# bridgedp/hunter_bipedal_control

Hardware: AMD Instinct MI355X
Metric: MPC+WBC updates/sec (batch=4096, N=100, 12-DoF) (higher is better)
Workload: dtype f64; 1 GPU; 4096 distinct hunter instances (4096/GPU, state seed 1234 + id), trot gait from t = 0.1, cmd_vel (0.3, 0, 0, 0), N=100 shooting intervals (dt 0.015 s), node tables generated on the device (hb_refgen_update, per-knot IK joint references), 1 SQP iteration + WeightedWbc per update, x0 of every call perturbed by measurement noise (sigma 0.01) so that no call re-solves a converged problem: every line s; batch_per_gpu=4096, total_instances=4096, horizon_nodes=100

## Files before the change

### hunter_bipedal_control_amd/abi.py

```python
from __future__ import annotations

import ctypes as C
from types import SimpleNamespace

import numpy as np

NX, NU, NV, NJ, NC, NBODY, NWBC, NRBD, SWING_REF = 22, 22, 16, 10, 4, 11, 38, 32, 6
FLY, MODE_R, MODE_L, STANCE = 0, 1, 2, 3
HB_PAYLOAD_SIZE = 10
HB_PROFILE_MAX_KNOTS = 16
HB_PROFILE_RECORD = 10


class HbModel(C.Structure):
    _fields_ = [
        ("parent", C.c_int32 * NJ),
        ("joint_origin", (C.c_double * 3) * NJ),
        ("joint_axis", (C.c_double * 3) * NJ),
        ("q_lower", C.c_double * NJ), ("q_upper", C.c_double * NJ),
        ("qd_limit", C.c_double * NJ), ("effort", C.c_double * NJ),
        ("mass", C.c_double * NBODY),
        ("com", (C.c_double * 3) * NBODY),
        ("inertia", (C.c_double * 6) * NBODY),
        ("contact_body", C.c_int32 * NC),
        ("contact_offset", (C.c_double * 3) * NC),
        ("gravity", C.c_double),
    ]


class HbConfig(C.Structure):
    _fields_ = [
        ("dt", C.c_double),
        ("sqp_iterations", C.c_int32), ("wbc_type", C.c_int32),
        ("g_max", C.c_double), ("g_min", C.c_double),
        ("alpha_decay", C.c_double), ("alpha_min", C.c_double), ("gamma_c", C.c_double), ("armijo_factor", C.c_double),
        ("Q_diag", C.c_double * NX),
        ("R_task_diag", C.c_double * 24),
        ("initial_state", C.c_double * NX),
        ("friction_mu", C.c_double), ("friction_reg", C.c_double), ("friction_gripper", C.c_double),
        ("friction_hess_shift", C.c_double),
        ("friction_barrier_mu", C.c_double), ("friction_barrier_delta", C.c_double),
        ("soft_swing_weight", C.c_double),
        ("pos_limit_barrier", C.c_double * 2), ("vel_limit_barrier", C.c_double * 2),
        ("force_limit_barrier", C.c_double * 2), ("force_limit", C.c_double * 2),
        ("position_error_gain", C.c_double),
        ("zero_vel_z_gain", C.c_double), ("zero_vel_z_offset", C.c_double),
        ("xy_ref_gain", C.c_double),
        ("torque_limits", C.c_double * 5),
        ("wbc_friction_mu", C.c_double),
        ("swing_kp", C.c_double), ("swing_kd", C.c_double),
        ("base_height_kp", C.c_double), ("base_height_kd", C.c_double),
        ("base_angular_kp", C.c_double), ("base_angular_kd", C.c_double),
        ("weight_swing_leg", C.c_double), ("weight_base_accel", C.c_double), ("weight_contact_force", C.c_double),
        ("wbc_eps_reg", C.c_double),
        ("wbc_max_iter", C.c_int32), ("reserved", C.c_int32),
        ("default_joint_state", C.c_double * NJ),
        ("delta_tol", C.c_double),
        ("wbc_reg_steps", C.c_int32), ("wbc_eps_mode", C.c_int32),
    ]


_LQ = dict(LQ_LOADS=10, LQ_LEG_VALUES=6, LQ_VALUE_PREPASS=7, LQ_DIRECTIONS=9, LQ_COMPOSE=1, LQ_FACTOR=2, LQ_SOLVES=3, LQ_DEFECT=30,
           LQ_B_COLUMNS=31, LQ_COST=4, LQ_SOFT_ROWS=5, LQ_Q=32, LQ_P=33, LQ_R=34)
_WBC = dict(WBC_A_BASE=13, WBC_A_LEGS=14, WBC_A_FINISH=15, WBC_A=11, WBC_B=12)
_RIC1 = dict(RIC1_STAGING=20, RIC1_GEMM1=21, RIC1_GEMM2=22, RIC1_FACTOR=23)
_RIC4 = dict(RIC4_STAGING=24, RIC4_GEMM1=25, RIC4_GEMM2=26, RIC4_FACTOR=27)
_HWBC = dict(HWBC_LEVEL0=41, HWBC_KERNEL0=43, HWBC_QP1=44, HWBC_LEVEL1=42)
FORMS = dict(NONE=0, **_LQ, **_WBC, **_RIC1, **_RIC4, **_HWBC, RIC_BWD_ONE=101, RIC_BWD_FOUR=104, RIC_FWD_ROW=111, RIC_FWD_WAVE=114,
             LQT_ONE_RECORD=117, LQT_TRACE=118, LQT_PARK_NOTHING=119, LQT_VALUES_ONCE=125, LQT_VALUES=126, LQT_VALUES_FWD=127,
             LQT_VALUES_LEGS=128, LQ_ONE_NODE=129, LS_EVAL_NODE=151, RIC1_TRACE=197, WBC_TRACE=198, RIC4_TRACE=199)
FORM_RANGES = dict(LQ_TRIP_POW2=(120, 124), LQ_TRIP_LEN=(131, 146))
FORM = SimpleNamespace(**FORMS)
LQ_STOPS, WBC_STOPS, RIC1_STOPS, RIC4_STOPS, HWBC_STOPS = (tuple(d.values()) for d in (_LQ, _WBC, _RIC1, _RIC4, _HWBC))


class HbStats(C.Structure):
    _fields_ = [
        ("ms_lq", C.c_double), ("ms_riccati_bwd", C.c_double), ("ms_riccati_fwd", C.c_double),
        ("ms_linesearch", C.c_double), ("ms_mpc_total", C.c_double), ("ms_wbc", C.c_double),
        ("n_mpc_solves", C.c_int64), ("n_wbc_solves", C.c_int64),
        ("n_status", C.c_int32 * 4),
    ]


def _fill(arr, values):
    a = np.asarray(values)
    if a.ndim == 1:
        for i, v in enumerate(a):
            arr[i] = v.item()
    else:
        for i in range(a.shape[0]):
            for j in range(a.shape[1]):
                arr[i][j] = a[i, j].item()


def make_model(params: dict) -> HbModel:
    m = params["model"]
    out = HbModel()
    for name in ("parent", "joint_origin", "joint_axis", "q_lower", "q_upper", "qd_limit", "effort", "mass", "com",
                 "inertia", "contact_body", "contact_offset"):
        _fill(getattr(out, name), m[name])
    out.gravity = m["gravity"]
    return out


def make_config(params: dict, **overrides) -> HbConfig:
    c = params["config"]
    out = HbConfig()
    out.dt = c["dt"]
    out.sqp_iterations = c["sqp_iterations"]
    out.wbc_type = 0
    out.g_max, out.g_min = c["g_max"], c["g_min"]
    out.alpha_decay, out.alpha_min, out.gamma_c, out.armijo_factor = 0.5, 1e-4, 1e-6, 1e-4
    _fill(out.Q_diag, c["Q_diag"])
    _fill(out.R_task_diag, c["R_task_diag"])
    _fill(out.initial_state, c["initial_state"])
    out.friction_mu = c["friction_mu"]
    out.friction_reg, out.friction_gripper, out.friction_hess_shift = 25.0, 0.0, 1e-6
    out.friction_barrier_mu, out.friction_barrier_delta = c["friction_barrier_mu"], c["friction_barrier_delta"]
    out.soft_swing_weight = c["soft_swing_weight"]
    _fill(out.pos_limit_barrier, [1.0, 0.1])
    _fill(out.vel_limit_barrier, [1.0, 0.1])
    _fill(out.force_limit_barrier, [0.1, 1.0])
    _fill(out.force_limit, [0.0, 350.0])
    out.position_error_gain = c["position_error_gain"]
    out.zero_vel_z_gain, out.zero_vel_z_offset = 3.0, -0.06
    out.xy_ref_gain = 3.0
    _fill(out.torque_limits, c["torque_limits"])
    out.wbc_friction_mu = c["wbc_friction_mu"]
    out.swing_kp, out.swing_kd = c["swing_kp"], c["swing_kd"]
    out.base_height_kp, out.base_height_kd = c["base_height_kp"], c["base_height_kd"]
    out.base_angular_kp, out.base_angular_kd = c["base_angular_kp"], c["base_angular_kd"]
    out.weight_swing_leg, out.weight_base_accel = c["weight_swing_leg"], c["weight_base_accel"]
    out.weight_contact_force = c["weight_contact_force"]
    out.wbc_eps_reg = 1e-8
    out.wbc_max_iter = 120
    _fill(out.default_joint_state, c["default_joint_state"])
    out.delta_tol = c["delta_tol"]
    out.wbc_reg_steps = 1
    for k, v in overrides.items():
        if isinstance(v, (list, tuple)):
            _fill(getattr(out, k), v)
        else:
            setattr(out, k, v)
    return out


class HbEstimatorConfig(C.Structure):
    _fields_ = [(k, C.c_double) for k in (
        "foot_radius", "imu_process_noise_position", "imu_process_noise_velocity", "foot_process_noise_position",
        "foot_sensor_noise_position", "foot_sensor_noise_velocity", "foot_height_sensor_noise",
        "contact_force_cutoff_frequency", "contact_threshold")]


def make_estimator_config(params: dict, **overrides) -> HbEstimatorConfig:
    out = HbEstimatorConfig()
    for k, _ in HbEstimatorConfig._fields_:
        setattr(out, k, overrides.get(k, params["config"]["kalman"][k]))
    return out


class HbSensorConfig(C.Structure):
    _fields_ = [(k, C.c_double) for k in ("orientation_noise", "gyro_noise", "accel_noise", "joint_pos_noise", "joint_vel_noise",
                                          "joint_torque_noise")] + [("seed", C.c_uint64), ("instance_offset", C.c_uint32),
                                                                    ("reserved", C.c_int32)]


def make_sensor_config(seed: int = 0, instance_offset: int = 0, **sigmas) -> HbSensorConfig:
    out = HbSensorConfig()
    names = [k for k, _ in HbSensorConfig._fields_[:6]]
    for k, v in sigmas.items():
        if k not in names:
            raise TypeError(f"make_sensor_config: unknown channel {k!r} (one of {names})")
        setattr(out, k, float(v))
    out.seed, out.instance_offset, out.reserved = int(seed) & 0xFFFFFFFFFFFFFFFF, int(instance_offset), 0
    return out


class HbContactConfig(C.Structure):
    _fields_ = [("mode", C.c_int32), ("sweeps", C.c_int32), ("mu", C.c_double), ("ground_z", C.c_double), ("erp", C.c_double),
                ("tol", C.c_double), ("fall_height", C.c_double), ("reserved", C.c_int32 * 2)]


HB_CONTACT_NONFINITE, HB_CONTACT_FALLEN, HB_CONTACT_UNCONVERGED = 1, 2, 4
CONTACT_DEFAULT_SWEEPS = 30


def make_contact_config(params: dict, **overrides) -> HbContactConfig:
    d = dict(mode=1, sweeps=CONTACT_DEFAULT_SWEEPS, mu=params["config"]["friction_mu"], ground_z=0.0, erp=0.2, tol=1e-3, fall_height=0.0)
    for k in overrides:
        if k not in d:
            raise TypeError(f"make_contact_config: unknown field {k!r} (one of {sorted(d)})")
    d.update(overrides)
    out = HbContactConfig()
    out.mode, out.sweeps = int(d["mode"]), int(d["sweeps"])
    for k in ("mu", "ground_z", "erp", "tol", "fall_height"):
        setattr(out, k, float(d[k]))
    return out


class HbJointModel(C.Structure):
    _fields_ = [(k, C.c_double * NJ) for k in ("armature", "damping", "frictionloss", "lower", "upper", "torque_limit")] + [
        ("limit_erp", C.c_double), ("tol", C.c_double), ("limits", C.c_int32), ("reserved", C.c_int32)]


HB_JOINT_UNCONVERGED = 1 << 30


def make_joint_model(params: dict, **overrides) -> HbJointModel:
    m = params["model"]
    d = dict(armature=0.1, damping=1.0, frictionloss=0.2, lower=m["q_lower"], upper=m["q_upper"], torque_limit=100.0, limit_erp=0.2,
             tol=1e-3, limits=1)
    for k in overrides:
        if k not in d:
            raise TypeError(f"make_joint_model: unknown field {k!r} (one of {sorted(d)})")
    d.update(overrides)
    out = HbJointModel()
    for k in ("armature", "damping", "frictionloss", "lower", "upper", "torque_limit"):
        _fill(getattr(out, k), np.broadcast_to(np.asarray(d[k], dtype=float), (NJ,)))
    out.limit_erp, out.tol, out.limits, out.reserved = float(d["limit_erp"]), float(d["tol"]), int(d["limits"]), 0
    return out


# ... 254 lines not shown
```

### hunter_bipedal_control_amd/csrc/hb_forms.hpp

```cpp
#pragma once

namespace hb {
namespace form {

#define HB_FORM_CODES(X) \
  X(NONE,             0, "decode_forms",                  "the product: every form picked by the number of instances in flight") \
   \
  X(LQ_LOADS,        10, "lq_node",                       "stop: loads") \
  X(LQ_LEG_VALUES,    6, "lq_node",                       "stop: + leg value pass") \
  X(LQ_VALUE_PREPASS, 7, "lq_node",                       "stop: + value pre-pass") \
  X(LQ_DIRECTIONS,    9, "lq_node_dense",                 "stop: + direction pass (k_lq_trip: read-back of the parked image + direction pass)") \
  X(LQ_COMPOSE,       1, "lq_tail",                       "stop: + compose") \
  X(LQ_FACTOR,        2, "lq_tail",                       "stop: + Gram matrix, pivoted Cholesky") \
  X(LQ_SOLVES,        3, "lq_tail",                       "stop: + solves") \
  X(LQ_DEFECT,       30, "lq_tail",                       "stop: + defect, A~ B~ tiles") \
  X(LQ_B_COLUMNS,    31, "lq_tail",                       "stop: + B~ columns, b~") \
  X(LQ_COST,          4, "lq_tail",                       "stop: + cost") \
  X(LQ_SOFT_ROWS,     5, "lq_tail",                       "stop: + soft rows, Pj, M") \
  X(LQ_Q,            32, "lq_tail",                       "stop: + Q~ q~") \
  X(LQ_P,            33, "lq_tail",                       "stop: + P~ r~") \
  X(LQ_R,            34, "lq_tail",                       "stop: + R~ (what is left: recovery data)") \
   \
  X(WBC_A_BASE,      13, "wbc_phase_a, wbc_solve",        "stop: phase A, base pass") \
  X(WBC_A_LEGS,      14, "wbc_phase_a, wbc_solve",        "stop: + leg passes") \
  X(WBC_A_FINISH,    15, "wbc_phase_a, wbc_solve",        "stop: + composition, desired base acceleration") \
  X(WBC_A,           11, "wbc_solve",                     "stop: phase A (rigid-body quantities and fills)") \
  X(WBC_B,           12, "wbc_solve",                     "stop: + phase B (cost factor, unconstrained minimiser)") \
   \
  X(RIC1_STAGING,    20, "k_ric_bwd",                     "stop: staging of the record only") \
  X(RIC1_GEMM1,      21, "ric_phase12, k_ric_bwd",        "stop: + GEMM 1") \
  X(RIC1_GEMM2,      22, "ric_phase12, k_ric_bwd",        "stop: + GEMM 2") \
  X(RIC1_FACTOR,     23, "riccati_bwd_node, k_ric_bwd",   "stop: + factor, solves (what is left: GEMM 3)") \
   \
  X(RIC4_STAGING,    24, "k_ric_bwd4, decode_forms",      "stop: staging only") \
  X(RIC4_GEMM1,      25, "k_ric_bwd4, decode_forms",      "stop: + GEMM 1") \
  X(RIC4_GEMM2,      26, "k_ric_bwd4, decode_forms",      "stop: + GEMM 2") \
  X(RIC4_FACTOR,     27, "k_ric_bwd4, decode_forms",      "stop: + factor, solves | first part of GEMM 3") \
   \
  X(HWBC_LEVEL0,     41, "k_hwbc",                        "stop: level 0") \
  X(HWBC_KERNEL0,    43, "hwbc_solve",                    "stop: + kernel basis of level 0") \
  X(HWBC_QP1,        44, "hwbc_solve",                    "stop: + level-1 QP") \
  X(HWBC_LEVEL1,     42, "k_hwbc",                        "stop: + kernel basis of level 1 (what is left: level 2)") \
   \
  X(RIC_BWD_ONE,    101, "decode_forms",                  "selector: one-wavefront backward sweep (k_ric_bwd)") \
  X(RIC_BWD_FOUR,   104, "decode_forms",                  "selector: four-wavefront backward sweep (k_ric_bwd4)") \
  X(RIC_FWD_ROW,    111, "decode_forms",                  "selector: row form of the forward sweep (k_ric_fwd)") \
  X(RIC_FWD_WAVE,   114, "decode_forms",                  "selector: wave form of the forward sweep (k_ric_fwd_w)") \
   \
  X(LQT_ONE_RECORD, 117, "k_lq_trip",                     "stop: every node of a workgroup writes one record slot (stores issued, lines stay in the L2)") \
  X(LQT_TRACE,      118, "k_lq_trip, lq_trip_values",     "trace (-DHB_LQV_TRACE): cycle counts of workgroup 1000's value phase; the kernel returns behind it") \
  X(LQT_PARK_NOTHING, 119, "lq_park_out",                 "stop: the value phase computes but parks nothing (stale data is read back)") \
  X(LQT_VALUES_ONCE, 125, "k_lq_trip",                    "stop: the value phase runs once per trip, later launches reuse what it parked") \
  X(LQT_VALUES,     126, "k_lq_trip",                     "stop: the value phase alone (first of LQT_VALUES .. LQT_VALUES_LEGS)") \
  X(LQT_VALUES_FWD, 127, "k_lq_trip, lq_trip_values",     "stop: the value phase up to its forward sweep") \
  X(LQT_VALUES_LEGS, 128, "k_lq_trip, lq_trip_values",    "stop: the value phase up to its leg pass (last of LQT_VALUES ..)") \
  X(LQ_ONE_NODE,    129, "decode_forms",                  "selector: the one-node-per-wavefront kernel k_lq (differs from the trips by rounding)") \
   \
  X(LS_EVAL_NODE,   151, "decode_forms",                  "selector: thread-per-node line-search evaluation (k_ls_eval_node, k_ls_tail_eval_node; differs from the two-lane form by rounding)") \
   \
  X(RIC1_TRACE,     197, "k_ric_bwd",                     "trace: cycle counts of stage 50 of instance 9") \
  X(WBC_TRACE,      198, "wbc_solve, decode_forms",       "trace: cycle counts of the WeightedWbc solve of instance 5 (leaves the sweep's choice alone)") \
  X(RIC4_TRACE,     199, "k_ric_bwd4, decode_forms",      "trace: cycle counts of stage 50 of instance 7")

#define HB_FORM_RANGES(X) \
  X(LQ_TRIP_POW2,   120, 124, "decode_forms",             "selector: LQ trips of 2^(value - first) nodes") \
  X(LQ_TRIP_LEN,    131, 146, "decode_forms",             "selector: LQ trips of value - first + 1 nodes (1 .. 16)")

enum Code : int {
#define HB_FORM_ENUM(id, value, reader, meaning) id = value,
#define HB_FORM_RANGE_ENUM(id, first, last, reader, meaning) id##_FIRST = first, id##_LAST = last,
  HB_FORM_CODES(HB_FORM_ENUM) HB_FORM_RANGES(HB_FORM_RANGE_ENUM)
#undef HB_FORM_ENUM
#undef HB_FORM_RANGE_ENUM
};

struct Entry { const char* name; int first, last; const char* reader; const char* meaning; };
constexpr Entry kTable[] = {
#define HB_FORM_ROW(id, value, reader, meaning) {#id, value, value, reader, meaning},
#define HB_FORM_RANGE_ROW(id, first, last, reader, meaning) {#id, first, last, reader, meaning},
  HB_FORM_CODES(HB_FORM_ROW) HB_FORM_RANGES(HB_FORM_RANGE_ROW)
#undef HB_FORM_ROW
#undef HB_FORM_RANGE_ROW
};

}

struct KernelForms {
  enum class Bwd { Auto, One, Four } bwd = Bwd::Auto;
  enum class Fwd { Auto, Row, Wave } fwd = Fwd::Auto;
  enum class Lq { Trips, OneNode } lq = Lq::Trips;
  enum class Ls { Pair, Node } ls = Ls::Pair;
  int trip_len = 0;
};

inline KernelForms decode_forms(int reserved, bool ablate) {
  using namespace form;
  KernelForms f;
  if (reserved == RIC_BWD_FOUR) f.bwd = KernelForms::Bwd::Four;
  else if (ablate && ((reserved >= RIC4_STAGING && reserved <= RIC4_FACTOR) || reserved == RIC4_TRACE)) f.bwd = KernelForms::Bwd::Four;
  else if (reserved == RIC_BWD_ONE) f.bwd = KernelForms::Bwd::One;
  else if (ablate && reserved != NONE && reserved != WBC_TRACE) f.bwd = KernelForms::Bwd::One;
  if (reserved == RIC_FWD_WAVE) f.fwd = KernelForms::Fwd::Wave;
  else if (reserved == RIC_FWD_ROW) f.fwd = KernelForms::Fwd::Row;
  if (reserved == LQ_ONE_NODE) f.lq = KernelForms::Lq::OneNode;
  if (reserved == LS_EVAL_NODE) f.ls = KernelForms::Ls::Node;
  if (reserved >= LQ_TRIP_POW2_FIRST && reserved <= LQ_TRIP_POW2_LAST) f.trip_len = 1 << (reserved - LQ_TRIP_POW2_FIRST);
  if (reserved >= LQ_TRIP_LEN_FIRST && reserved <= LQ_TRIP_LEN_LAST) f.trip_len = reserved - LQ_TRIP_LEN_FIRST + 1;
  return f;
}

constexpr int kRicBwd4MaxBatch = 512;
inline bool use_ric_bwd4(const KernelForms& f, int concurrent) {
  return f.bwd == KernelForms::Bwd::Four || (f.bwd == KernelForms::Bwd::Auto && concurrent <= kRicBwd4MaxBatch);
}

constexpr int kRicFwdWaveMaxBatch = 512;
inline bool use_ric_fwd_wave(const KernelForms& f, int concurrent) {
  return f.fwd == KernelForms::Fwd::Wave || (f.fwd == KernelForms::Fwd::Auto && concurrent <= kRicFwdWaveMaxBatch);
}

inline bool use_ground_forms(bool map_in_force) { return map_in_force; }

struct PlantForm {
  enum class Ground { Pinned, Level, Terrain, Varied, Profile } ground;
  bool joints, hybrid;
};
inline PlantForm plant_form(int contact_mode, bool joints_on, bool terrain_on, bool modelvar_on, bool profile_on, bool hybrid) {
  using G = PlantForm::Ground;
  if (contact_mode != 1) return {G::Pinned, false, hybrid};
  return {profile_on ? G::Profile : modelvar_on ? G::Varied : terrain_on ? G::Terrain : G::Level, joints_on, hybrid};
}

constexpr int kLqTripsPerSlot = 4;
inline int lq_trip_len(const KernelForms& f, int concurrent, int Nmax, int n_cu) {
  if (f.trip_len) return f.trip_len;
  const long slots = 12L * n_cu;
  for (int sh = 4; sh > 0; --sh)
    if (long(concurrent) * ((Nmax + (1 << sh) - 1) >> sh) >= kLqTripsPerSlot * slots) return 1 << sh;
  return 1;
}

}
```

### hunter_bipedal_control_amd/csrc/hb_qpfactor.hpp

```cpp
#pragma once
#include "hb_math.hpp"

namespace hb {

template <int N>
HB_HD double dot4(const double* a, int sa, const double* b, int sb) {
  double s[4] = {0.0, 0.0, 0.0, 0.0};
#pragma unroll
  for (int i = 0; i < N; ++i) s[i & 3] += a[i * sa] * b[i * sb];
  return (s[0] + s[1]) + (s[2] + s[3]);
}

template <class Ctx>
HB_HD void givens_insert_row(const Ctx& cx, double* R, int ld, int n, double* np) {
  for (int k = 0; k < n; ++k) {
    const double a = R[k * ld + k], b = np[k];
    cx.sync();
    if (b != 0.0) {
      const double rh = rsqrt_t(a * a + b * b), cc = a * rh, ss = b * rh;
      for (int j = k + cx.lane; j < n; j += cx.nlanes) {
        const double t1 = R[k * ld + j], t2 = np[j];
        R[k * ld + j] = cc * t1 + ss * t2;
        np[j] = -ss * t1 + cc * t2;
      }
    }
    cx.sync();
  }
}

struct UniformDiag {
  double se, se2;
  HB_HD explicit UniformDiag(double s) : se(s), se2(s * s) {}
  HB_HD double at(int) const { return se; }
  HB_HD double plus_sq(int, double x) const { return se2 + x; }
  HB_HD double minus_sq(int, double x) const { return x - se2; }
};
struct HeadTailDiag {
  double head, tail;
  int n_head;
  HB_HD double at(int k) const { return k < n_head ? head : tail; }
  HB_HD double plus_sq(int k, double x) const { return fma(at(k), at(k), x); }
  HB_HD double minus_sq(int k, double x) const { return fma(-at(k), at(k), x); }
};

#if defined(__HIP_DEVICE_COMPILE__)
template <int MA, class Diag>
__device__ __forceinline__ double householder_factor(double (&acol)[MA], int j, int n, int wstore, const Diag& D, double* R, int ld) {
  double diag = 0.0;
#pragma unroll 1
  for (int k = 0; k < n; ++k) {
    double dot = 0.0;
    double ck[MA];
#pragma unroll
    for (int r = 0; r < MA; ++r) {
      ck[r] = wave_bcast_f64(acol[r], k);
      dot += ck[r] * acol[r];
    }
    const double se = D.at(k);
    const double sig2 = D.plus_sq(k, wave_bcast_f64(dot, k));
    const double alpha = -sqrt(sig2);
    const double v0 = se - alpha;
    const double beta = 2.0 * rcp_t(D.minus_sq(k, sig2) + v0 * v0);
    const double w = beta * (dot + (j == k ? v0 * se : 0.0));
    const bool live = j > k && j < n;
#pragma unroll
    for (int r = 0; r < MA; ++r) acol[r] = live ? acol[r] - w * ck[r] : (j == k ? 0.0 : acol[r]);
    if (j < wstore) R[k * ld + j] = (j < k || j >= n) ? 0.0 : (j == k ? alpha : -w * v0);
    if (j == k) diag = alpha;
  }
  return diag;
}
#endif

template <int MA, bool kGrad, class Ctx, class Diag>
HB_HD void regularised_factor(const Ctx& cx, int n, int mA, const double* A, int lda, const double* b, double* g, const Diag& D, double* R,
                              int ld, int wstore, double* np) {
#if defined(__HIP_DEVICE_COMPILE__)
  const int j = cx.lane;
  double acol[MA];
  double gj = 0.0;
#pragma unroll
  for (int r = 0; r < MA; ++r) {
    acol[r] = (j < n && r < mA) ? A[r * lda + j] : 0.0;
    if constexpr (kGrad) gj += acol[r] * (r < mA ? b[r] : 0.0);
  }
  if (kGrad && j < n) g[j] = gj;
  householder_factor<MA>(acol, j, n, wstore, D, R, ld);
  (void)np;
  cx.sync();
#else
  for (int idx = cx.lane; idx < n * wstore; idx += cx.nlanes) {
    const int i = idx / wstore, c = idx % wstore;
    R[i * ld + c] = i == c ? D.at(i) : 0.0;
  }
  if constexpr (kGrad)
    for (int i = cx.lane; i < n; i += cx.nlanes) g[i] = 0.0;
  cx.sync();
  for (int rw = 0; rw < mA; ++rw) {
    for (int j = cx.lane; j < n; j += cx.nlanes) {
      np[j] = A[rw * lda + j];
      if constexpr (kGrad) g[j] += A[rw * lda + j] * b[rw];
    }
    cx.sync();
    givens_insert_row(cx, R, ld, n, np);
  }
#endif
}

template <class Ctx>
HB_HD void invert_upper(const Ctx& cx, const double* R, int ld, int n, double* J) {
  for (int col = cx.lane; col < n; col += cx.nlanes) {
    for (int i = n - 1; i > col; --i) J[i * ld + col] = 0.0;
    for (int i = col; i >= 0; --i) {
      double s = (i == col) ? 1.0 : 0.0;
      for (int k = i + 1; k <= col; ++k) s = fma(-R[i * ld + k], J[k * ld + col], s);
      J[i * ld + col] = s * rcp_t(R[i * ld + i]);
    }
  }
  cx.sync();
}

template <class Ctx>
HB_HD void drop_constraint(const Ctx& cx, int n, int ld, double* R, double* J, int* act, double* lam, int* is_active, int l, int& q) {
  if (cx.lane == 0) is_active[act[l]] = 0;
  cx.sync();
  for (int j = l; j < q - 1; ++j) {
    for (int i = cx.lane; i <= j + 1; i += cx.nlanes) R[i * ld + j] = R[i * ld + j + 1];
    if (cx.lane == 0) { act[j] = act[j + 1]; lam[j] = lam[j + 1]; }
    cx.sync();
  }
  for (int i = cx.lane; i < q; i += cx.nlanes) R[i * ld + q - 1] = 0.0;
  --q;
  cx.sync();
  for (int j = l; j < q; ++j) {
    const double a = R[j * ld + j], b = R[(j + 1) * ld + j];
    cx.sync();
    if (b != 0.0) {
      const double rh = rsqrt_t(a * a + b * b), cc = a * rh, ss = b * rh;
      for (int k = cx.lane; k < n; k += cx.nlanes) {
        if (k >= j && k < q) {
          const double t1 = R[j * ld + k], t2 = R[(j + 1) * ld + k];
          R[j * ld + k] = cc * t1 + ss * t2;
          R[(j + 1) * ld + k] = -ss * t1 + cc * t2;
        }
        const double u1 = J[k * ld + j], u2 = J[k * ld + j + 1];
        J[k * ld + j] = cc * u1 + ss * u2;
        J[k * ld + j + 1] = -ss * u1 + cc * u2;
      }
    }
    cx.sync();
    if (cx.lane == 0) R[(j + 1) * ld + j] = 0.0;
    cx.sync();
  }
}

}
```

### hunter_bipedal_control_amd/csrc/hb_wbc.hpp

```cpp
#pragma once
#include "hb_lq.hpp"
#include "hb_qpfactor.hpp"

namespace hb {

constexpr int NW = HB_NWBC;

struct WbcBatch {
  int B;
  double* t_now;
  double* rbd;
  int* walk;
  double* xdes;
  double* udes;
  int* mode;
  int* stance;
  double* sol;
  int* status;
  int* iters;
  double* px;
  double* pu;
  double* pt;
  int* pmode;
  int* pn;
// ... 628 lines not shown

template <class Ctx>
HB_HD double wbc_eps(const Ctx& cx, const DevConfig& C, const WbcWork& W, const WbcState& st) {
  if (C.wbc_eps_mode != 1) return C.wbc_eps;
  double part = 0.0;
  for (int e = cx.lane; e < 256; e += cx.nlanes) {
    const int i = e >> 4, j = e & 15;
    double g = 0.0;
    for (int rw = 0; rw < st.n_aw; ++rw) g += W.Aw[rw * 16 + i] * W.Aw[rw * 16 + j];
    part += g * g;
  }
  W.red[cx.lane] = part;
  cx.sync();
  double h2 = st.stance_mode ? 0.0 : 12.0 * (C.w_force * C.w_force) * (C.w_force * C.w_force);
  for (int l = 0; l < cx.nlanes; ++l) h2 += W.red[l];
  cx.sync();
  const double e1 = sqrt(h2) * (1.0e3 * 2.220446049250313e-16);
  return e1 > 0.0 ? e1 : C.wbc_eps;
}

template <class Ctx>
HB_HD void wbc_invert_cost_factor(const Ctx& cx, const WbcWork& W) {
#if defined(__HIP_DEVICE_COMPILE__)
  if (cx.lane < NW) {
    const int col = cx.lane;
    if (col >= 16) {
      W.J[col * NW + col] = rcp_t(W.R[col * NW + col]);
    } else {
      double xc[16];
#pragma unroll
      for (int i = 15; i >= 0; --i) {
        double s = (i == col) ? 1.0 : 0.0;
#pragma unroll
        for (int k = i + 1; k < 16; ++k) s -= W.R[i * NW + k] * (k <= col ? xc[k] : 0.0);
        xc[i] = i <= col ? s * rcp_t(W.R[i * NW + i]) : 0.0;
      }
#pragma unroll
      for (int i = 0; i < 16; ++i)
        if (i <= col) W.J[i * NW + col] = xc[i];
    }
  }
#else
  invert_upper(cx, W.R, NW, 16, W.J);
  for (int col = 16 + cx.lane; col < NW; col += cx.nlanes) W.J[col * NW + col] = rcp_t(W.R[col * NW + col]);
#endif
  cx.sync();
}

template <class Ctx>
HB_HD void wbc_cost_factor(const Ctx& cx, const DevConfig& C, const double* udes, const WbcWork& W, WbcState& st) {
  const double se = sqrt(st.eps);
  for (int idx = cx.lane; idx < NW * NW; idx += cx.nlanes) W.R[idx] = (idx / NW == idx % NW) ? se : 0.0;
  cx.sync();
  if (!st.stance_mode && C.w_force != 0.0) {
    for (int i = cx.lane; i < 12; i += cx.nlanes) W.R[(16 + i) * NW + 16 + i] = sqrt(st.eps + C.w_force * C.w_force);
    cx.sync();
  }
  for (int i = cx.lane; i < NW; i += cx.nlanes) {
    double s = 0.0;
    if (i < 16)
      for (int rw = 0; rw < st.n_aw; ++rw) s += W.Aw[rw * 16 + i] * W.bw[rw];
    else if (i < 28 && !st.stance_mode)
      s = C.w_force * C.w_force * udes[i - 16];
    W.d[i] = s;
  }
  regularised_factor<18, false>(cx, 16, st.n_aw, W.Aw, 16, nullptr, nullptr, UniformDiag(se), W.R, NW, 16, W.np);
  HB_WBC_MARK(2)
  for (int idx = cx.lane; idx < NW * NW; idx += cx.nlanes) W.J[idx] = 0.0;
  cx.sync();
  wbc_invert_cost_factor(cx, W);
  for (int k = cx.lane; k < NW; k += cx.nlanes) W.z[k] = dot4<NW>(W.J + k, NW, W.d, 1);
  cx.sync();
  for (int i = cx.lane; i < NW; i += cx.nlanes) W.x[i] = dot4<NW>(W.J + i * NW, 1, W.z, 1);
  for (int idx = cx.lane; idx < NW * NW; idx += cx.nlanes) W.R[idx] = 0.0;
  for (int i = cx.lane; i < 64; i += cx.nlanes) W.is_active[i] = 0;
  cx.sync();
  HB_WBC_MARK(3)
}

template <class Ctx>
HB_HD void wbc_load_jrow(const Ctx& cx, const WbcWork& W, WbcState& st) {
#if defined(__HIP_DEVICE_COMPILE__)
#pragma unroll
  for (int j = 0; j < NW; ++j) st.jrow[j] = cx.lane < NW ? W.J[cx.lane * NW + j] : 0.0;
#endif
}

HB_HD double wbc_j2d2(const WbcWork& W, const WbcState& st, int i) {
  double sa[4] = {0.0, 0.0, 0.0, 0.0};
#pragma unroll
  for (int j = 0; j < NW; ++j) {
#if defined(__HIP_DEVICE_COMPILE__)
    const double jij = st.jrow[j];
#else
    const double jij = W.J[i * NW + j];
#endif
    sa[j & 3] += jij * (j >= st.q ? W.d[j] : 0.0);
  }
  return (sa[0] + sa[1]) + (sa[2] + sa[3]);
}

template <class Ctx>
HB_HD void wbc_reflect(const Ctx& cx, const WbcWork& W, WbcState& st, int q) {
  double* d = W.d;
  double nrm2 = 0.0;
#if defined(__HIP_DEVICE_COMPILE__)
  {
    const double dj = (cx.lane >= q && cx.lane < NW) ? d[cx.lane] : 0.0;
    nrm2 = wave_sum_f64(dj * dj);
  }
#else
  for (int j = q; j < NW; ++j) nrm2 += d[j] * d[j];
#endif
  const double dq = d[q];
  const double alpha = dq > 0.0 ? -sqrt(nrm2) : sqrt(nrm2);
  const double v0 = dq - alpha;
  const double vtv = nrm2 - dq * dq + v0 * v0;
  if (vtv > 0.0 && nrm2 > 0.0) {
    const double beta = 2.0 * rcp_t(vtv);
    for (int k = cx.lane; k < NW; k += cx.nlanes) {
#if defined(__HIP_DEVICE_COMPILE__)
      double* row = st.jrow;
#else
      double row[NW];
#pragma unroll
      for (int j = 0; j < NW; ++j) row[j] = W.J[k * NW + j];
#endif
      double sa[4] = {0.0, 0.0, 0.0, 0.0};
#pragma unroll
      for (int j = 0; j < NW; ++j) sa[j & 3] += row[j] * (j < q ? 0.0 : (j == q ? v0 : d[j]));
      const double sacc = ((sa[0] + sa[1]) + (sa[2] + sa[3])) * beta;
#pragma unroll
      for (int j = 0; j < NW; ++j) {
        row[j] = row[j] - sacc * (j < q ? 0.0 : (j == q ? v0 : d[j]));
        W.J[k * NW + j] = row[j];
      }
    }
  }
  cx.sync();
  for (int j = q + cx.lane; j < NW; j += cx.nlanes) d[j] = (j == q) ? alpha : 0.0;
  cx.sync();
}

template <class Ctx>
HB_HD bool wbc_append_row(const Ctx& cx, const WbcWork& W, WbcState& st, int p, double lam_p) {
  if (!(fabs(W.d[st.q]) > 1e-13 * fmax(1.0, fabs(W.R[0])))) return false;
  for (int i = cx.lane; i <= st.q; i += cx.nlanes) W.R[i * NW + st.q] = W.d[i];
  if (cx.lane == 0) { W.act[st.q] = p; W.lam[st.q] = lam_p; W.is_active[p] = 1; }
  ++st.q;
  return true;
}

template <class Ctx>
HB_HD void wbc_equality_block(const Ctx& cx, const DevConfig& C, const WbcWork& W, WbcState& st) {
  const WbcCons& wc = st.wc;
  if (wc.n_eq > C.wbc_max_iter) st.status = HB_INST_MAXITER;
#if defined(__HIP_DEVICE_COMPILE__)
#pragma unroll
#endif
  for (int p = 0; p < 16 + 3 * HB_NC; ++p) {
    if (p >= wc.n_eq || st.status != 0) break;
    if (p == 5) { HB_WBC_MARK(7) }
    if (p < 16) {
      for (int k = cx.lane; k < NW; k += cx.nlanes) W.d[k] = dot4<NW>(W.J + k, NW, W.Ee + p * NW, 1);
    } else {
      const int sidx = 16 + 3 * wc.swing_foot((p - 16) / 3) + (p - 16) % 3;
      for (int k = cx.lane; k < NW; k += cx.nlanes) W.d[k] = W.J[sidx * NW + k];
    }
    cx.sync();
    if (p == 5) { HB_WBC_MARK(8) }
    wbc_reflect(cx, W, st, st.q);
    if (p == 5) { HB_WBC_MARK(9) }
    if (!wbc_append_row(cx, W, st, p, 0.0)) { st.status = HB_INST_INFEASIBLE; break; }
    ++st.iter;
    cx.sync();
  }
  HB_WBC_MARK(4)
  const int q = st.q;
  if (st.status == 0 && q > 0) {
    for (int pp = cx.lane; pp < NW; pp += cx.nlanes) {
      double sres = 0.0;
      if (pp < q) {
        if (pp < 16) sres = dot4<NW>(W.Ee + pp * NW, 1, W.x, 1) - W.beom[pp];
        else sres = W.x[16 + 3 * wc.swing_foot((pp - 16) / 3) + (pp - 16) % 3];
      }
      W.r[pp] = sres;
    }
    cx.sync();
#if defined(__HIP_DEVICE_COMPILE__)
    {
      double sres = cx.lane < NW ? W.r[cx.lane] : 0.0;
      const double rdiag = rcp_t(cx.lane < q ? W.R[cx.lane * NW + cx.lane] : 1.0);
      double xacc = 0.0;
      for (int i = 0; i < q; ++i) {
        const double yi = wave_bcast_f64(sres * rdiag, i);
        if (cx.lane > i && cx.lane < q) sres -= W.R[i * NW + cx.lane] * yi;
        xacc += (cx.lane < NW ? W.J[cx.lane * NW + i] : 0.0) * yi;
      }
      if (cx.lane < NW) W.x[cx.lane] -= xacc;
    }
#else
    for (int l0 = cx.lane; l0 < 1; l0 += cx.nlanes) {
      for (int i = 0; i < q; ++i) {
        const double yi = W.r[i] / W.R[i * NW + i];
        for (int pp = i + 1; pp < q; ++pp) W.r[pp] -= W.R[i * NW + pp] * yi;
        W.r[i] = yi;
      }
      for (int k = 0; k < NW; ++k) {
        double acc = 0.0;
        for (int i = 0; i < q; ++i) acc += W.J[k * NW + i] * W.r[i];
        W.x[k] -= acc;
      }
    }
#endif
    cx.sync();
  }
  HB_WBC_MARK(5)
  st.n_eq_active = q;
}

template <class Ctx, class Visit>
HB_HD void wbc_backsolve_inequalities(const Ctx& cx, const WbcWork& W, const WbcState& st, Visit visit) {
  for (int i = st.q - 1; i >= st.n_eq_active; --i) {
    const double ri = W.r[i] / W.R[i * NW + i];
    cx.sync();
    for (int k = st.n_eq_active + cx.lane; k < i; k += cx.nlanes) W.r[k] -= W.R[k * NW + i] * ri;
    if (cx.lane == 0) visit(i, ri);
    cx.sync();
  }
}

template <class Ctx>
HB_HD void wbc_regularisation_step(const Ctx& cx, const WbcWork& W, WbcState& st) {
  for (int i = cx.lane; i < NW; i += cx.nlanes) { W.np[i] = W.x[i] - W.xb[i]; W.xb[i] = W.x[i]; }
  cx.sync();
  for (int k = cx.lane; k < NW; k += cx.nlanes) W.d[k] = dot4<NW>(W.J + k, NW, W.np, 1);
  cx.sync();
  for (int i = cx.lane; i < NW; i += cx.nlanes) {
    W.x[i] += st.eps * wbc_j2d2(W, st, i);
    if (i < st.q) W.r[i] = W.d[i];
  }
  cx.sync();
  wbc_backsolve_inequalities(cx, W, st, [&](int i, double ri) { W.lam[i] = fmax(0.0, W.lam[i] + st.eps * ri); });
}

template <class Ctx>
HB_HD int wbc_most_violated(const Ctx& cx, const DevConfig& C, const WbcWork& W, const WbcState& st) {
  double best = 0.0;
  int bi = -1;
  for (int c = st.wc.n_eq + cx.lane; c < st.wc.n_eq + st.wc.n_in; c += cx.nlanes) {
    if (W.is_active[c]) continue;
    int idx[3];
    double cfv[3], rhs;
    const int nn = sparse_row(st.wc, C, c, idx, cfv, &rhs);
    double s = -rhs;
    for (int t = 0; t < nn; ++t) s += cfv[t] * W.x[idx[t]];
    if (s > 1e-9 * fmax(1.0, fabs(rhs)) && s > best) { best = s; bi = c; }
  }
#if defined(__HIP_DEVICE_COMPILE__)
  const double gb = wave_max_f64(best);
  if (!(gb > 0.0)) return -1;
  return __builtin_amdgcn_readlane(bi, __ffsll(__ballot(best == gb)) - 1);
#else
  W.red[cx.lane] = best;
  cx.sync();
  double gb = 0.0;
  int gl = -1;
  for (int l = 0; l < cx.nlanes; ++l)
    if (W.red[l] > gb) { gb = W.red[l]; gl = l; }
  cx.sync();
  if (gl < 0) return -1;
  if (cx.lane == gl) W.misc[1] = double(bi);
  cx.sync();
  const int p = int(W.misc[1]);
  cx.sync();
  return p;
#endif
}

template <class Ctx>
HB_HD void wbc_inequalities(const Ctx& cx, const DevConfig& C, const WbcWork& W, WbcState& st) {
  const double inf = 1e300;
  double* x = W.x;
  double* d = W.d;
  double* z = W.z;
  double* r = W.r;
  double* lam = W.lam;
  while (st.status == 0) {
    const int p = wbc_most_violated(cx, C, W, st);
    if (p < 0) break;
    double prhs;
    int pidx[3] = {0, 0, 0};
    double pcf[3] = {0.0, 0.0, 0.0};
    const int pnn = sparse_row(st.wc, C, p, pidx, pcf, &prhs);
    const int pi0 = pidx[0], pi1 = pnn > 1 ? pidx[1] : pidx[0];
    const double pc0 = pcf[0], pc1 = pnn > 1 ? pcf[1] : 0.0;
    double lam_p = 0.0;
    bool done_p = false;
    while (!done_p) {
      if (++st.iter > C.wbc_max_iter) { st.status = HB_INST_MAXITER; break; }
      for (int k = cx.lane; k < NW; k += cx.nlanes) d[k] = pc0 * W.J[pi0 * NW + k] + pc1 * W.J[pi1 * NW + k];
      cx.sync();
      const double sp = pc0 * x[pi0] + pc1 * x[pi1] - prhs;
      for (int i = cx.lane; i < NW; i += cx.nlanes) {
        z[i] = wbc_j2d2(W, st, i);
        if (i < st.q) r[i] = d[i];
      }
      cx.sync();
      const int q = st.q, n_eq_active = st.n_eq_active;
      const bool need_r = q > n_eq_active;
      if (need_r) wbc_backsolve_inequalities(cx, W, st, [&](int i, double ri) { r[i] = ri; });
      const double zn = pc0 * z[pi0] + pc1 * z[pi1], nn2 = pc0 * pc0 + pc1 * pc1;
      const double t2 = (zn > 1e-14 * (1.0 + nn2)) ? sp * rcp_t(zn) : inf;
      const double dir = 1.0;
      double t1 = inf;
      int l = -1;
      for (int j = n_eq_active; j < q && need_r; ++j) {
        const double rj = dir * r[j];
        if (rj > 0.0) {
          const double tj = lam[j] / rj;
          if (tj < t1) { t1 = tj; l = j; }
        }
      }
      const double t2abs = fabs(t2);
      const double t = fmin(t1, t2abs);
      if (t >= inf) { st.status = HB_INST_INFEASIBLE; break; }
      cx.sync();
      if (t2 >= inf) {
        if (need_r)
          for (int j = n_eq_active + cx.lane; j < q; j += cx.nlanes) lam[j] -= t * dir * r[j];
        lam_p += t;
      } else {
        for (int k = cx.lane; k < NW; k += cx.nlanes) x[k] -= dir * t * z[k];
        if (need_r)
          for (int j = n_eq_active + cx.lane; j < q; j += cx.nlanes) lam[j] -= t * dir * r[j];
        lam_p += t;
      }
      cx.sync();
      if (t2 < inf && t == t2abs) {
        wbc_reflect(cx, W, st, q);
        wbc_append_row(cx, W, st, p, lam_p);
        cx.sync();
        done_p = true;
      } else {
        drop_constraint(cx, NW, NW, W.R, W.J, W.act, lam, W.is_active, l, st.q);
        wbc_load_jrow(cx, W, st);
      }
    }
  }
}

template <class Ctx, bool kCert = false>
HB_HD void wbc_solve(const Ctx& cx, const DevModel& M, const DevConfig& C, const double* xdes, const double* udes,
                     const double* rbd, int mode, bool stance_mode, double* lds, double* sol, int* status_out,
                     int* iters_out, double* cert = nullptr, double* dual = nullptr) {
  const WbcWork W(lds);
  WbcState st;
  HB_WBC_MARK(0)
  st.wc = wbc_cons_of_mode(mode);
  st.stance_mode = stance_mode;
  st.n_aw = stance_mode ? 6 : 3 * st.wc.n_sw + 6;
  static_assert(PHASE_A_WORK_DOUBLES <= NW * NW, "phase-A workspace must fit the J buffer");
  wbc_phase_a(cx, M, C, xdes, udes, rbd, st.wc, stance_mode, C.w_swing, C.w_base, W.R, W.Ee, W.beom, W.Aw, W.bw, nullptr, nullptr, W.J);
  if (cx.lane == 0) W.misc[0] = 0.0;
  cx.sync();
  HB_WBC_MARK(1)
  HB_ABLATE_STOP(C.debug_stop == form::WBC_A || (C.debug_stop >= form::WBC_A_BASE && C.debug_stop <= form::WBC_A_FINISH));
  st.eps = wbc_eps(cx, C, W, st);
  wbc_cost_factor(cx, C, udes, W, st);
  HB_ABLATE_STOP(C.debug_stop == form::WBC_B);
  wbc_load_jrow(cx, W, st);
  wbc_equality_block(cx, C, W, st);
  for (int i = cx.lane; i < NW; i += cx.nlanes) W.xb[i] = 0.0;
  cx.sync();
  const int n_reg = C.wbc_reg_steps > 0 ? C.wbc_reg_steps : 0;
  for (int phase = 0; phase <= n_reg && st.status == 0; ++phase) {
    if (phase > 0) wbc_regularisation_step(cx, W, st);
    wbc_inequalities(cx, C, W, st);
  }
  cx.sync();
  HB_WBC_MARK(6)
#if defined(HB_ABLATE) && defined(__HIP_DEVICE_COMPILE__)
  if (C.debug_stop == form::WBC_TRACE && blockIdx.x == 5 && cx.lane == 0)
    printf("wbc trace: phase A %lld | Householder of A_w %lld | J = R^-1, x0 %lld | equality block (%d rows) %lld | primal update %lld | inequalities (%d iterations) %lld | row 5: d = J'n %lld, reflector %lld  (cycles)\n",
           st.wt_[1] - st.wt_[0], st.wt_[2] - st.wt_[1], st.wt_[3] - st.wt_[2], st.n_eq_active, st.wt_[4] - st.wt_[3], st.wt_[5] - st.wt_[4], st.iter - st.n_eq_active, st.wt_[6] - st.wt_[5], st.wt_[8] - st.wt_[7], st.wt_[9] - st.wt_[8]);
#endif
  if (st.status == 0)
    for (int i = cx.lane; i < NW; i += cx.nlanes) sol[i] = W.x[i];
  if (cx.lane == 0) {
    *status_out = st.status;
    *iters_out = st.iter;
  }
  if constexpr (kCert) wbc_certificate(cx, C, st.wc, udes, stance_mode, st.n_aw, st.eps, st.status, W, sol, cert, dual);
}

HB_HD void policy_eval(const DevConfig& C, int n, const double* t, const double* px, const double* pu, const int* pmode, double tn,
                       const double* rbd, bool walk, double* xdes, double* udes, int* mode, int* stance) {
  if (!walk) {
    for (int i = 0; i < HB_NX; ++i) xdes[i] = 0.0;
    for (int i = 0; i < HB_NU; ++i) udes[i] = 0.0;
    for (int i = 0; i < 3; ++i) {
      xdes[6 + i] = rbd[3 + i];
      xdes[9 + i] = rbd[i];
    }
    for (int j = 0; j < HB_NJ; ++j) xdes[12 + j] = C.default_joint_state[j];
    *mode = 3;
    *stance = 1;
    return;
  }
  int k = 0;
  while (k < n - 1 && tn >= t[k + 1]) ++k;
  double a = (tn - t[k]) / (t[k + 1] - t[k]);
  a = fmin(1.0, fmax(0.0, a));
  for (int i = 0; i < HB_NX; ++i) xdes[i] = (1.0 - a) * px[k * HB_NX + i] + a * px[(k + 1) * HB_NX + i];
  const int k1 = (k + 1 < n) ? k + 1 : k;
  for (int i = 0; i < HB_NU; ++i) udes[i] = (1.0 - a) * pu[k * HB_NU + i] + a * pu[k1 * HB_NU + i];
  *mode = pmode[k];
  *stance = 0;
}

#if defined(__HIPCC__)
__global__ void k_policy_eval(WbcBatch w, int Nmax, const DevConfig* __restrict__ C) {
  const int inst = blockIdx.x * blockDim.x + threadIdx.x;
  if (inst >= w.B) return;
  policy_eval(*C, w.pn[inst], w.pt + size_t(inst) * (Nmax + 1), w.px + size_t(inst) * (Nmax + 1) * HB_NX,
              w.pu + size_t(inst) * Nmax * HB_NU, w.pmode + size_t(inst) * Nmax, w.t_now[inst], w.rbd + size_t(inst) * HB_NRBD,
              w.walk[inst] != 0, w.xdes + size_t(inst) * HB_NX, w.udes + size_t(inst) * HB_NU, w.mode + inst, w.stance + inst);
}

struct WbcDeviceCtx {
  int lane;
  static constexpr int nlanes = 64;
  __device__ WbcDeviceCtx() : lane(threadIdx.x) {}
  __device__ void sync() const {
    __builtin_amdgcn_fence(__ATOMIC_ACQ_REL, "wavefront");
    __builtin_amdgcn_wave_barrier();
  }
};

__global__ __launch_bounds__(64) void k_wbc(WbcBatch w, const DevModel* __restrict__ M, const DevConfig* __restrict__ C) {
  __builtin_amdgcn_s_setprio(3);
  const int inst = blockIdx.x;
  __shared__ double lds[WbcLds::total];
  wbc_solve(WbcDeviceCtx(), *M, *C, w.xdes + size_t(inst) * HB_NX, w.udes + size_t(inst) * HB_NU, w.rbd + size_t(inst) * HB_NRBD,
            w.mode[inst], w.stance[inst] != 0, lds, w.sol + size_t(inst) * NW, w.status + inst, w.iters + inst);
}

__global__ __launch_bounds__(64) void k_wbc_cert(WbcBatch w, const DevModel* __restrict__ M, const DevConfig* __restrict__ C,
                                                 double* cert, double* dual) {
  __builtin_amdgcn_s_setprio(3);
  const int inst = blockIdx.x;
  __shared__ double lds[WbcLds::total];
  wbc_solve<WbcDeviceCtx, true>(WbcDeviceCtx(), *M, *C, w.xdes + size_t(inst) * HB_NX, w.udes + size_t(inst) * HB_NU,
                                w.rbd + size_t(inst) * HB_NRBD, w.mode[inst], w.stance[inst] != 0, lds, w.sol + size_t(inst) * NW,
                                w.status + inst, w.iters + inst, cert + size_t(inst) * HB_WBC_CERT_SIZE,
                                dual + size_t(inst) * HB_WBC_NCONS_MAX);
}

__global__ void k_rbd(int n, const DevModel* __restrict__ M, const double* rbd, double* Mo, double* nle, double* J, double* dJv) {
  const int i = blockIdx.x * blockDim.x + threadIdx.x;
  if (i >= n) return;
  const double* rb = rbd + size_t(i) * HB_NRBD;
  double q[HB_NV], v[HB_NV];
  for (int a = 0; a < 3; ++a) { q[a] = rb[3 + a]; q[3 + a] = rb[a]; v[a] = rb[HB_NV + 3 + a]; }
  for (int j = 0; j < HB_NJ; ++j) { q[6 + j] = rb[6 + j]; v[6 + j] = rb[HB_NV + 6 + j]; }
  double sz, cz, sy, cy;
  sincos_t(q[3], sz, cz);
  sincos_t(q[4], sy, cy);
  const Vec3<double> er = euler_rates_from_omega<double>(sz, cz, sy, cy, Vec3<double>(rb[HB_NV], rb[HB_NV + 1], rb[HB_NV + 2]));
  v[3] = er.x; v[4] = er.y; v[5] = er.z;
  BodyPass P;
  body_pass(*M, q, v, P);
  mass_matrix(P, Mo + size_t(i) * 256);
  for (int a = 0; a < 16; ++a) nle[size_t(i) * 16 + a] = P.nle[a];
  for (int ci = 0; ci < HB_NC; ++ci) {
    for (int col = 0; col < 16; ++col) {
      const Vec3<double> jc = contact_jac(P, ci, col);
      J[(size_t(i) * 12 + 3 * ci + 0) * 16 + col] = jc.x;
      J[(size_t(i) * 12 + 3 * ci + 1) * 16 + col] = jc.y;
      J[(size_t(i) * 12 + 3 * ci + 2) * 16 + col] = jc.z;
    }
    dJv[size_t(i) * 12 + 3 * ci + 0] = P.foot_acc[ci].x;
    dJv[size_t(i) * 12 + 3 * ci + 1] = P.foot_acc[ci].y;
    dJv[size_t(i) * 12 + 3 * ci + 2] = P.foot_acc[ci].z;
  }
}
#endif

}
```

Baseline: 544,100 updates/s.

## Replace row-by-row WBC equality updates with one blocked Householder QR

```diff
diff --git a/hunter_bipedal_control_amd/abi.py b/hunter_bipedal_control_amd/abi.py
--- a/hunter_bipedal_control_amd/abi.py
+++ b/hunter_bipedal_control_amd/abi.py
@@ -68,7 +68,7 @@
 _HWBC = dict(HWBC_LEVEL0=41, HWBC_KERNEL0=43, HWBC_QP1=44, HWBC_LEVEL1=42)
 FORMS = dict(NONE=0, **_LQ, **_WBC, **_RIC1, **_RIC4, **_HWBC, RIC_BWD_ONE=101, RIC_BWD_FOUR=104, RIC_FWD_ROW=111, RIC_FWD_WAVE=114,
              LQT_ONE_RECORD=117, LQT_TRACE=118, LQT_PARK_NOTHING=119, LQT_VALUES_ONCE=125, LQT_VALUES=126, LQT_VALUES_FWD=127,
-             LQT_VALUES_LEGS=128, LQ_ONE_NODE=129, LS_EVAL_NODE=151, RIC1_TRACE=197, WBC_TRACE=198, RIC4_TRACE=199)
+             LQT_VALUES_LEGS=128, LQ_ONE_NODE=129, LS_EVAL_NODE=151, WBC_EQ_ROWS=161, RIC1_TRACE=197, WBC_TRACE=198, RIC4_TRACE=199)
 FORM_RANGES = dict(LQ_TRIP_POW2=(120, 124), LQ_TRIP_LEN=(131, 146))
 FORM = SimpleNamespace(**FORMS)
 LQ_STOPS, WBC_STOPS, RIC1_STOPS, RIC4_STOPS, HWBC_STOPS = (tuple(d.values()) for d in (_LQ, _WBC, _RIC1, _RIC4, _HWBC))
diff --git a/hunter_bipedal_control_amd/csrc/hb_forms.hpp b/hunter_bipedal_control_amd/csrc/hb_forms.hpp
--- a/hunter_bipedal_control_amd/csrc/hb_forms.hpp
+++ b/hunter_bipedal_control_amd/csrc/hb_forms.hpp
@@ -57,6 +57,8 @@
   X(LQ_ONE_NODE,    129, "decode_forms",                  "selector: the one-node-per-wavefront kernel k_lq (differs from the trips by rounding)") \
    \
   X(LS_EVAL_NODE,   151, "decode_forms",                  "selector: thread-per-node line-search evaluation (k_ls_eval_node, k_ls_tail_eval_node; differs from the two-lane form by rounding)") \
+   \
+  X(WBC_EQ_ROWS,    161, "wbc_solve",                     "selector: equality rows of k_wbc enter one by one (d = J'n and J <- J H per row; differs from the blocked QR by rounding)") \
    \
   X(RIC1_TRACE,     197, "k_ric_bwd",                     "trace: cycle counts of stage 50 of instance 9") \
   X(WBC_TRACE,      198, "wbc_solve, decode_forms",       "trace: cycle counts of the WeightedWbc solve of instance 5 (leaves the sweep's choice alone)") \
diff --git a/hunter_bipedal_control_amd/csrc/hb_qpfactor.hpp b/hunter_bipedal_control_amd/csrc/hb_qpfactor.hpp
--- a/hunter_bipedal_control_amd/csrc/hb_qpfactor.hpp
+++ b/hunter_bipedal_control_amd/csrc/hb_qpfactor.hpp
@@ -1,4 +1,5 @@
 #pragma once
+#include <type_traits>
 #include "hb_math.hpp"
 
 namespace hb {
@@ -71,6 +72,47 @@
   return diag;
 }
 #endif
+
+template <int P0, int P1, class F>
+HB_HD void static_steps(F&& f) {
+  if constexpr (P0 < P1) {
+    if (f(std::integral_constant<int, P0>())) static_steps<P0 + 1, P1>(f);
+  }
+}
+
+struct Reflector { double v0, beta, alpha; };
+template <int N>
+HB_HD Reflector householder_vector(const double* c, int sc, int p) {
+  double s[4] = {0.0, 0.0, 0.0, 0.0};
+#pragma unroll
+  for (int j = 0; j < N; ++j) {
+    const double cj = j >= p ? c[j * sc] : 0.0;
+    s[j & 3] += cj * cj;
+  }
+  const double nrm2 = (s[0] + s[1]) + (s[2] + s[3]);
+  const double cp = c[p * sc];
+  const double alpha = cp > 0.0 ? -sqrt(nrm2) : sqrt(nrm2);
+  const double v0 = cp - alpha;
+  const double vtv = nrm2 - cp * cp + v0 * v0;
+  Reflector h = {v0, 0.0, alpha};
+  if (vtv > 0.0 && nrm2 > 0.0) h.beta = 2.0 * rcp_t(vtv);
+  return h;
+}
+template <int N>
+HB_HD void householder_apply(const double* v, int sv, double v0, double beta, int p, double* c, int sc) {
+  double s[4] = {0.0, 0.0, 0.0, 0.0};
+#pragma unroll
+  for (int j = 0; j < N; ++j) {
+    const double vj = j < p ? 0.0 : (j == p ? v0 : v[j * sv]);
+    s[j & 3] += c[j * sc] * vj;
+  }
+  const double w = ((s[0] + s[1]) + (s[2] + s[3])) * beta;
+#pragma unroll
+  for (int j = 0; j < N; ++j) {
+    const double vj = j < p ? 0.0 : (j == p ? v0 : v[j * sv]);
+    c[j * sc] = c[j * sc] - w * vj;
+  }
+}
 
 template <int MA, bool kGrad, class Ctx, class Diag>
 HB_HD void regularised_factor(const Ctx& cx, int n, int mA, const double* A, int lda, const double* b, double* g, const Diag& D, double* R,
diff --git a/hunter_bipedal_control_amd/csrc/hb_wbc.hpp b/hunter_bipedal_control_amd/csrc/hb_wbc.hpp
--- a/hunter_bipedal_control_amd/csrc/hb_wbc.hpp
+++ b/hunter_bipedal_control_amd/csrc/hb_wbc.hpp
@@ -804,15 +804,13 @@
 }
 
 template <class Ctx>
-HB_HD void wbc_equality_block(const Ctx& cx, const DevConfig& C, const WbcWork& W, WbcState& st) {
+HB_HD void wbc_equality_rows(const Ctx& cx, const WbcWork& W, WbcState& st) {
   const WbcCons& wc = st.wc;
-  if (wc.n_eq > C.wbc_max_iter) st.status = HB_INST_MAXITER;
 #if defined(__HIP_DEVICE_COMPILE__)
 #pragma unroll
 #endif
   for (int p = 0; p < 16 + 3 * HB_NC; ++p) {
     if (p >= wc.n_eq || st.status != 0) break;
-    if (p == 5) { HB_WBC_MARK(7) }
     if (p < 16) {
       for (int k = cx.lane; k < NW; k += cx.nlanes) W.d[k] = dot4<NW>(W.J + k, NW, W.Ee + p * NW, 1);
     } else {
@@ -820,12 +818,115 @@
       for (int k = cx.lane; k < NW; k += cx.nlanes) W.d[k] = W.J[sidx * NW + k];
     }
     cx.sync();
-    if (p == 5) { HB_WBC_MARK(8) }
     wbc_reflect(cx, W, st, st.q);
-    if (p == 5) { HB_WBC_MARK(9) }
     if (!wbc_append_row(cx, W, st, p, 0.0)) { st.status = HB_INST_INFEASIBLE; break; }
     ++st.iter;
     cx.sync();
+  }
+}
+
+template <class Ctx>
+HB_HD void wbc_equality_qr(const Ctx& cx, const DevConfig& C, const WbcWork& W, WbcState& st) {
+  const WbcCons& wc = st.wc;
+  const int n_eq = wc.n_eq;
+  HB_WBC_MARK(7)
+  {
+    WaveTile<3, 1> t;
+    tile_init(cx, t, NW, 16, [](int, int) { return 0.0; });
+    tile_mma<40, NW, true, NW, true, NW>(cx, t, W.J, W.Ee, NW, 16);
+    tile_store_rm<NW>(cx, t, NW, 16, W.R);
+  }
+  cx.sync();
+#if defined(__HIP_DEVICE_COMPILE__)
+  {
+    const int c = cx.lane, s = c < 16 ? 0 : c - 16;
+    const bool own = c < n_eq;
+    const double* src = !own ? W.R : (c < 16 ? W.R + c : W.J + (16 + 3 * wc.swing_foot(s / 3) + s % 3) * NW);
+    const int ss = !own ? 0 : (c < 16 ? NW : 1);
+#pragma unroll
+    for (int j = 0; j < NW; ++j) st.jrow[j] = own ? src[j * ss] : 0.0;
+  }
+#else
+  for (int c = 16 + cx.lane; c < n_eq; c += cx.nlanes) {
+    const int sidx = 16 + 3 * wc.swing_foot((c - 16) / 3) + (c - 16) % 3;
+    for (int j = 0; j < NW; ++j) W.R[j * NW + c] = W.J[sidx * NW + j];
+  }
+#endif
+  cx.sync();
+  int n_ref = 0;
+  double r00 = 0.0;
+  constexpr int NE = 16 + 3 * HB_NC;
+  static_steps<0, NE>([&](auto pc) {
+    constexpr int p = decltype(pc)::value;
+    if (p >= n_eq) return false;
+#if defined(__HIP_DEVICE_COMPILE__)
+    if (cx.lane == p) {
+      const Reflector h = householder_vector<NW>(st.jrow, 1, p);
+#pragma unroll
+      for (int j = 0; j < NW; ++j) W.R[j * NW + p] = j == p ? h.alpha : st.jrow[j];
+      W.z[p] = h.v0; W.np[p] = h.beta; W.d[p] = h.alpha;
+    }
+#else
+    for (int c = p + cx.lane; c == p; c += cx.nlanes) {
+      const Reflector h = householder_vector<NW>(W.R + p, NW, p);
+      W.R[p * NW + p] = h.alpha;
+      W.z[p] = h.v0; W.np[p] = h.beta; W.d[p] = h.alpha;
+    }
+#endif
+    cx.sync();
+    const double v0 = W.z[p], beta = W.np[p], alpha = W.d[p];
+    n_ref = p + 1;
+    if (!(fabs(alpha) > 1e-13 * fmax(1.0, fabs(r00)))) { st.status = HB_INST_INFEASIBLE; return false; }
+    if (p == 0) r00 = alpha;
+    if (beta != 0.0) {
+#if defined(__HIP_DEVICE_COMPILE__)
+      if (cx.lane > p && cx.lane < n_eq) householder_apply<NW>(W.R + p, NW, v0, beta, p, st.jrow, 1);
+#else
+      for (int c = p + 1 + cx.lane; c < n_eq; c += cx.nlanes) householder_apply<NW>(W.R + p, NW, v0, beta, p, W.R + c, NW);
+#endif
+    }
+    if (cx.lane == 0) { W.act[p] = p; W.lam[p] = 0.0; W.is_active[p] = 1; }
+    ++st.q;
+    ++st.iter;
+    return true;
+  });
+  HB_WBC_MARK(8)
+#if defined(__HIP_DEVICE_COMPILE__)
+  wbc_load_jrow(cx, W, st);
+  static_steps<0, NE>([&](auto pc) {
+    constexpr int p = decltype(pc)::value;
+    if (p >= n_ref) return false;
+    const double v0 = W.z[p], beta = W.np[p];
+    if (beta != 0.0) householder_apply<NW>(W.R + p, NW, v0, beta, p, st.jrow, 1);
+    return true;
+  });
+  if (cx.lane < NW) {
+#pragma unroll
+    for (int j = 0; j < NW; ++j) W.J[cx.lane * NW + j] = st.jrow[j];
+  }
+#else
+  for (int k = cx.lane; k < NW; k += cx.nlanes)
+    for (int p = 0; p < n_ref; ++p)
+      if (W.np[p] != 0.0) householder_apply<NW>(W.R + p, NW, W.z[p], W.np[p], p, W.J + k * NW, 1);
+#endif
+  cx.sync();
+  for (int idx = cx.lane; idx < NW * NE; idx += cx.nlanes) {
+    const int i = idx / NE, c = idx - NE * i;
+    if (i > c || c >= st.q) W.R[i * NW + c] = 0.0;
+  }
+  cx.sync();
+  HB_WBC_MARK(9)
+}
+
+template <class Ctx>
+HB_HD void wbc_equality_block(const Ctx& cx, const DevConfig& C, const WbcWork& W, WbcState& st) {
+  const WbcCons& wc = st.wc;
+  if (wc.n_eq > C.wbc_max_iter) st.status = HB_INST_MAXITER;
+  if (C.debug_stop == form::WBC_EQ_ROWS) {
+    wbc_load_jrow(cx, W, st);
+    wbc_equality_rows(cx, W, st);
+  } else if (st.status == 0) {
+    wbc_equality_qr(cx, C, W, st);
   }
   HB_WBC_MARK(4)
   const int q = st.q;
@@ -1021,7 +1122,6 @@
   st.eps = wbc_eps(cx, C, W, st);
   wbc_cost_factor(cx, C, udes, W, st);
   HB_ABLATE_STOP(C.debug_stop == form::WBC_B);
-  wbc_load_jrow(cx, W, st);
   wbc_equality_block(cx, C, W, st);
   for (int i = cx.lane; i < NW; i += cx.nlanes) W.xb[i] = 0.0;
   cx.sync();
@@ -1034,7 +1134,7 @@
   HB_WBC_MARK(6)
 #if defined(HB_ABLATE) && defined(__HIP_DEVICE_COMPILE__)
   if (C.debug_stop == form::WBC_TRACE && blockIdx.x == 5 && cx.lane == 0)
-    printf("wbc trace: phase A %lld | Householder of A_w %lld | J = R^-1, x0 %lld | equality block (%d rows) %lld | primal update %lld | inequalities (%d iterations) %lld | row 5: d = J'n %lld, reflector %lld  (cycles)\n",
+    printf("wbc trace: phase A %lld | Householder of A_w %lld | J = R^-1, x0 %lld | equality block (%d rows) %lld | primal update %lld | inequalities (%d iterations) %lld | of the block: D0 and its QR %lld, reflectors over J %lld  (cycles)\n",
            st.wt_[1] - st.wt_[0], st.wt_[2] - st.wt_[1], st.wt_[3] - st.wt_[2], st.n_eq_active, st.wt_[4] - st.wt_[3], st.wt_[5] - st.wt_[4], st.iter - st.n_eq_active, st.wt_[6] - st.wt_[5], st.wt_[8] - st.wt_[7], st.wt_[9] - st.wt_[8]);
 #endif
   if (st.status == 0)
```

Result: no change. 547,900 updates/s (median of 6 runs) (+0.7%).
